# KIYOYOZU/SPH-Poiseuille-Flow

Hardware: AMD Instinct MI355X
Metric: particle-steps/s (higher is better)
Workload: dtype f64; 1 GPU; C2: dp=0.025, DL=3.0, DH=1.0, n_fluid=4800, n_wall=960, n_total=5760, c_f=15.0, transport_coeff=0.3; start=developed (analytic parabola + 0.05dp jitter, seed 12345); lanes_per_particle=16, steps_per_graph=40, rebuild_every=16, forced_rebuilds=0, parallelism=1 GPU, device-resident loop, hipGraph replay

## Files before the change

### sph-poiseuille-flow_amd/csrc/sphx_kernels.hpp

```cpp
#pragma once
#include <type_traits>

#include "sphx_device.hpp"

namespace sphx {

constexpr int kBlock = 256;
constexpr int kScanBlock = 1024;
constexpr int kBigScanCells = 8192;

struct Grid {
    int ncx, ncy, ncells;
    int periodic;
    double DL, half_DL;
    double x0, y0, inv_csx, inv_csy;
    double own_lo, own_hi;
    int own_by_cell, own_c0, own_c1;
};

__device__ __forceinline__ bool owns(const Grid &g, double x, int cell)
{
    if (!g.own_by_cell) return x >= g.own_lo && x < g.own_hi;
    const int cx = cell / g.ncy;
    return cx >= g.own_c0 && cx < g.own_c1;
// ... 38 lines not shown
    double *drhon;
    double4 *a;
    double4 *B;
    double2 *fp, *f;
    double *rho_out, *p_out;
    int *cellid, *count, *perm, *src_of;
    double *vpart;
    double *dpart;
    int *nl_idx;
    int *nl_cnt;
    int *flags;
    int *tile_sum;
    int nl_stride, nl_cap;
    int *sl_idx, *sl_cnt;
    int sl_cap;
    double sl_rcut2;
    int cap;
    int n_vpart;
    double half_skin;
    double *vol;
    int *nl_pk, *sl_pk;
    int has_slack;
    double *seal_out;
    int lazy_out;
    int *tmap;
};

constexpr unsigned long long kVpartEmpty = ~0ull;

struct Walls {
    const double2 *pos;
    const double4 *a;
    const int *id;
    const int *start;
    const int *row_any;
    int n;
};

struct Members {
    Clock *clk;
    const Phys *ph;
    long long part;
    int cells;
    int blocks;
    int lanes;
    long long list, slist;
};

template <typename T>
__device__ __forceinline__ T *member_ptr(T *p, long long stride, int m)
{
    return p ? p + stride * m : p;
}

__device__ __forceinline__ FluidSet member_set(const Members &mb, int m, FluidSet s)
{
    s.pos = member_ptr(s.pos, mb.part, m); s.vel = member_ptr(s.vel, mb.part, m);
    s.drho = member_ptr(s.drho, mb.part, m); s.mass = member_ptr(s.mass, mb.part, m);
    s.id = member_ptr(s.id, mb.part, m); s.cell = member_ptr(s.cell, mb.part, m); s.posb = member_ptr(s.posb, mb.part, m);
    s.start = member_ptr(s.start, mb.cells, m);
    return s;
}

__device__ __forceinline__ FluidTmp member_tmp(const Members &mb, int m, FluidTmp t)
{
    const long long P = mb.part;
    t.posn = member_ptr(t.posn, P, m); t.veln = member_ptr(t.veln, P, m); t.drhon = member_ptr(t.drhon, P, m);
    t.a = member_ptr(t.a, P, m); t.B = member_ptr(t.B, P, m); t.fp = member_ptr(t.fp, P, m); t.f = member_ptr(t.f, P, m);
    t.rho_out = member_ptr(t.rho_out, P, m); t.p_out = member_ptr(t.p_out, P, m); t.vol = member_ptr(t.vol, P, m);
    t.cellid = member_ptr(t.cellid, P, m); t.perm = member_ptr(t.perm, P, m); t.src_of = member_ptr(t.src_of, P, m);
    t.count = member_ptr(t.count, (long long)mb.cells, m);
    t.vpart = member_ptr(t.vpart, (long long)mb.blocks, m); t.dpart = member_ptr(t.dpart, (long long)mb.blocks, m);
    t.nl_idx = member_ptr(t.nl_idx, mb.list, m); t.sl_idx = member_ptr(t.sl_idx, mb.slist, m);
    t.nl_cnt = member_ptr(t.nl_cnt, (long long)mb.lanes, m); t.sl_cnt = member_ptr(t.sl_cnt, (long long)mb.lanes, m);
    t.flags = member_ptr(t.flags, 1ll, m);
    t.tile_sum = nullptr;
    return t;
}

__device__ __forceinline__ void cell_of(const Grid &g, double x, double y, int &cx, int &cy)
{
    cx = (int)floor((x - g.x0) * g.inv_csx);
    cx = min(max(cx, 0), g.ncx - 1);
    cy = (int)floor((y - g.y0) * g.inv_csy);
    cy = min(max(cy, 0), g.ncy - 1);
}

// ... 58 lines not shown
__device__ __forceinline__ double dpp_f64(double v)
{
    const int lo = __builtin_amdgcn_mov_dpp(__double2loint(v), CTRL, 0xF, 0xF, true);
    const int hi = __builtin_amdgcn_mov_dpp(__double2hiint(v), CTRL, 0xF, 0xF, true);
    return __hiloint2double(hi, lo);
}
__device__ __forceinline__ double wave_max(double v)
{
    v = fmax(v, dpp_f64<0xB1>(v));
    v = fmax(v, dpp_f64<0x4E>(v));
    v = fmax(v, dpp_f64<0x141>(v));
    v = fmax(v, dpp_f64<0x140>(v));
    v = fmax(v, __shfl_xor(v, 16));
    return fmax(v, __shfl_xor(v, 32));
}
template <int LPP, bool MAX>
__device__ __forceinline__ int group_extreme(int v)
{
    auto pick = [](int a, int b) { return MAX ? max(a, b) : min(a, b); };
    if (LPP >= 2) v = pick(v, __builtin_amdgcn_mov_dpp(v, 0xB1, 0xF, 0xF, true));
    if (LPP >= 4) v = pick(v, __builtin_amdgcn_mov_dpp(v, 0x4E, 0xF, 0xF, true));
    if (LPP >= 8) v = pick(v, __builtin_amdgcn_mov_dpp(v, 0x141, 0xF, 0xF, true));
    if (LPP >= 16) v = pick(v, __builtin_amdgcn_mov_dpp(v, 0x140, 0xF, 0xF, true));
#pragma unroll
    for (int off = LPP / 2; off >= 16; off >>= 1) v = pick(v, __shfl_xor(v, off));
    return v;
}
template <int LPP>
__device__ __forceinline__ double group_sum(double v)
{
// ... 1 lines not shown
    if (LPP >= 4) v += dpp_f64<0x4E>(v);
    if (LPP >= 8) v += dpp_f64<0x141>(v);
    if (LPP >= 16) v += dpp_f64<0x140>(v);
#pragma unroll
    for (int off = LPP / 2; off >= 16; off >>= 1) v += __shfl_xor(v, off);
    return v;
}

__device__ __forceinline__ double tracked_drift2(const Grid &g, const FluidSet &s, int i, double xo, double yo, const double2 pb)
{
    if (g.own_by_cell && !owns(g, 0.0, s.cell[i])) return 0.0;
    const double ddx = min_image(g, xo - pb.x), ddy = yo - pb.y;
    const double d2 = ddx * ddx + ddy * ddy;
    return d2 != d2 ? INFINITY : d2;
}
__device__ __forceinline__ void store_block_drift(const FluidTmp &t, int blk, double d2)
{
    d2 = wave_max(d2);
    __shared__ double s_d2[kBlock / 64];
    if ((threadIdx.x & 63) == 0) s_d2[threadIdx.x >> 6] = d2;
    __syncthreads();
    if (threadIdx.x == 0) {
        double m = s_d2[0];
        for (int k = 1; k < kBlock / 64; ++k) m = fmax(m, s_d2[k]);
        t.dpart[blk] = m;
    }
}

template <int LPP, typename Body>
__device__ __forceinline__ void sweep(const Grid &g, const int *__restrict__ start, int cx, int cy,
                                      int sub, Body &&body)
{
    const int cylo = max(cy - 1, 0), cyhi = min(cy + 1, g.ncy - 1);
#pragma unroll
    for (int ox = -1; ox <= 1; ++ox) {
        int col;
        if (!neighbour_column(g, cx, ox, col)) continue;
        const int base = col * g.ncy;
        const int lo = start[base + cylo], hi = start[base + cyhi + 1];
        for (int k = lo + sub; k < hi; k += LPP) body(k);
// ... 556 lines not shown
    const double4 ai = in_cap ? t.a[i] : make_double4(1.0, 0.0, 0.0, 0.0);
    const double4 Bi = in_cap ? t.B[i] : make_double4(1.0, 0.0, 0.0, 1.0);
    const double mi = in_cap ? s.mass[i] : 1.0;
    const int nn_all = list_rows(kRowsAhead<LPP> ? head.packed : t.nl_cnt[tid]);
    const FirstRows<LPP> first = kRowsAhead<LPP> ? FirstRows<LPP>(head.e0, head.e1) : FirstRows<LPP>(t.nl_idx, t.nl_stride, tid);
    const bool tracked = s.posb != nullptr;
    const double2 pb = (tracked && in_cap && sub == 0) ? s.posb[i] : make_double2(0.0, 0.0);
    const double2 fp_own = (later && in_cap) ? t.fp[i] : make_double2(0.0, 0.0);
    const double2 p_now = (later && in_cap && sub == 0) ? t.posn[i] : make_double2(0.0, 0.0);
    const double dt = kRowsAhead<LPP> ? head.dt : clk->dt;
    const int run_q = kRowsAhead<LPP> ? head.run : clk->run[q], n_now = kRowsAhead<LPP> ? head.n : clk->n;
    if (kRowsAhead<LPP>) requests_issued();
    if (!run_q) return;
    const bool active = i < n_now;
    const double h = ph.kc.h;
    double ax = 0.0, ay = 0.0, ix = 0.0, iy = 0.0, px = 0.0, py = 0.0, d2 = 0.0;
    const double xi = pi.x, yi = pi.y, vxi = vi.x, vyi = vi.y;
    const double Voli = ai.x, p_i = ai.y, rhoh_i = ai.z;
    const double b11i = Bi.x, b12i = Bi.y, b21i = Bi.z, b22i = Bi.w;
    int first_wall = 1 << 20;
    int h_cell = -1;
    double2 pj0 = make_double2(0.0, 0.0), pj1 = pj0;
    double4 aj0 = make_double4(0.0, 0.0, 0.0, 0.0), aj1 = aj0;
    auto fluid_term = [&](const double2 pj, const double2 vj, const double4 aj, const double4 Bj) {
        const auto [r, ex, ey] = pair_geom(min_image(g, xi - pj.x), yi - pj.y);
        const double dW = spline_dW_in(ph.kc, r);
        const double Volj = aj.x;
        const double tx = (b11i + Bj.x) * ex + (b12i + Bj.y) * ey;
        const double ty = (b21i + Bj.z) * ex + (b22i + Bj.w) * ey;
        const double eBe = ex * tx + ey * ty;
        const double vxj = vj.x, vyj = vj.y;
// ... 92 lines not shown
    }
    px = group_sum<LPP>(px);
    py = group_sum<LPP>(py);
    if (active && sub == 0) {
        const double fx = px * Voli, fy = py * Voli;
        const double vxn = vxi + (fpx + fx) * inv_m * dt;
        const double vyn = vyi + (fpy + fy) * inv_m * dt;
        double sx = 0.0, sy = 0.0;
        if (!later) transport_shift(ix, iy, h, ph.tc, sx, sy);
        double xo = later ? p_now.x : xi + sx, yo = later ? p_now.y : yi + sy;
        xo += 0.5 * dt * vxi;
        yo += 0.5 * dt * vyi;
        xo += 0.5 * dt * vxn;
        yo += 0.5 * dt * vyn;
        if (tracked) d2 = tracked_drift2(g, s, i, xo, yo, pb);
        t.posn[i] = make_double2(g.periodic ? wrap_x(xo, ph.DL) : xo, yo);
        t.veln[i] = make_double2(vxn, vyn);
        if (!later) t.fp[i] = make_double2(fpx, fpy);
        t.f[i] = make_double2(fx, fy);
        if (HIST) {
            int cx, cy;
            cell_of(g, g.periodic ? wrap_x(xo, ph.DL) : xo, yo, cx, cy);
            h_cell = cx * g.ncy + cy;
            t.cellid[i] = h_cell;
            if (!rebin_near(g, c_binned, h_cell)) atomicOr(t.flags, 1);
        }
    }
    __shared__ int s_hc[HIST ? kBlock / LPP : 1];
    if (HIST && sub == 0) s_hc[threadIdx.x / LPP] = h_cell;
    store_block_drift(t, blk, d2);
    if (HIST && threadIdx.x < kBlock / LPP) {
        const int c = s_hc[threadIdx.x];
        int same = 0;
        bool first = true;
#pragma unroll
        for (int k = 0; k < kBlock / LPP; ++k) {
            const bool eq = s_hc[k] == c;
            same += eq ? 1 : 0;
            if (eq && k < (int)threadIdx.x) first = false;
        }
        if (c >= 0 && first) atomicAdd(&t.count[c], same);
    }
}
template <int LPP>
__global__ __launch_bounds__(kBlock) void k_forces(const Clock *clk, int q, int shape, int *nl_cnt, int *nl_idx, int nl_stride, int cap,
// ... 751 lines not shown
        const double sx = ph.tc * h * h * lim * ix, sy = ph.tc * h * h * lim * iy;
        double xo = xi + sx, yo = yi + sy;
        xo += 0.5 * dt * vxi;
        yo += 0.5 * dt * vyi;
        xo += 0.5 * dt * vxn;
        yo += 0.5 * dt * vyn;
        if (tracked) d2 = tracked_drift2(g, s, i, xo, yo, pb);
        if (g.periodic) xo = xo >= ph.DL ? xo - ph.DL : (xo < 0.0 ? xo + ph.DL : xo);
        t.posn[i] = make_double2(xo, yo);
        t.veln[i] = make_double2(vxn, vyn);
        if (want_out) {
            t.fp[i] = make_double2(fpx, fpy);
            t.f[i] = make_double2(fx, fy);
        }
    }
    store_block_drift(t, blk, d2);
}

template <int NT>
__device__ __forceinline__ int block_exclusive_scan_t(int v, int &total, int *s_wave )
{
    const int lane = threadIdx.x & 63, wave = threadIdx.x >> 6;
    int inc = v;
#pragma unroll
    for (int off = 1; off < 64; off <<= 1) {
        const int o = __shfl_up(inc, off);
        if (lane >= off) inc += o;
    }
    if (lane == 63) s_wave[wave] = inc;
    __syncthreads();
    if (wave == 0) {
// ... 38 lines not shown
    c.t += c.n_in > 1 ? c.dt * c.n_in : c.dt;
    c.dt_last = c.dt;
    c.step += 1;
    if (c.steps_left > 0) c.steps_left -= 1;
    if (!(c.vmax == c.vmax) || isinf(c.vmax)) c.status = SPHX_ERR_DIVERGED;
    if (flags) c.status = SPHX_ERR_GRID;
    if (n_new >= 0) c.n = n_new;
    c.dt = next_dt(c, ph);
    const int go = loop_continues(c) ? 1 : 0;
    if (q == 0) c.run[1] = go;
    else c.run[0] = go;
    *clk = c;
    if (!go && c.pub) *c.pub = c;
}

__device__ __forceinline__ void continuity_tail(Clock *clk, int q, const Phys &ph, const FluidTmp &t, int nb, int rebuilt = 0)
{
    if (!clk->run[q]) {
        if (threadIdx.x == 0) clk->run[1 - q] = 0;
        return;
    }
    Clock c0;
    int fl = 0;
    if (threadIdx.x == 0) { c0 = *clk; fl = *t.flags; }
    double m = 0.0, d = 0.0;
    int lost = 0;
    const bool track = t.half_skin >= 0.0;
    for (int k = threadIdx.x; k < nb; k += kBlock) {
        if (track) d = fmax(d, t.dpart[k]);
        unsigned long long *slot = reinterpret_cast<unsigned long long *>(&t.vpart[k]);
// ... 43 lines not shown
    m = wave_max(m);
    d = wave_max(d);
    lost = __any(lost) ? 1 : 0;
    __shared__ double s_m[kBlock / 64], s_d[kBlock / 64];
    __shared__ int s_l[kBlock / 64];
    if ((threadIdx.x & 63) == 0) { s_m[threadIdx.x >> 6] = m; s_d[threadIdx.x >> 6] = d; s_l[threadIdx.x >> 6] = lost; }
    __syncthreads();
    if (threadIdx.x == 0) {
        for (int k = 1; k < kBlock / 64; ++k) { m = fmax(m, s_m[k]); d = fmax(d, s_d[k]); lost |= s_l[k]; }
        t.seal_out[0] = lost ? INFINITY : sqrt(m);
        t.seal_out[1] = sqrt(d);
    }
}

constexpr int kFoldAhead = 8;
struct FoldRebin {
    static constexpr int kPer = kFoldCells / kBlock;
    int cnew = 0, id = 0, cold = 0, lo[3] = {0, 0, 0}, n[3] = {0, 0, 0}, hist[kPer], ccell[kFoldAhead], cid[kFoldAhead];
    double mass = 0.0;
    __device__ __forceinline__ int candidates() const { return n[0] + n[1] + n[2]; }
    __device__ __forceinline__ int slot(int v) const { return ranges_index(lo[0], lo[1], lo[2], n[0], n[1], v); }
};
__device__ __forceinline__ void fold_load(FoldRebin &r, const Grid &g, const FluidSet &s, const FluidTmp &t, int i, bool in_cap, bool lead)
{
    r.cnew = in_cap ? t.cellid[i] : 0;
    r.id = in_cap ? s.id[i] : 0;
    r.cold = lead ? s.cell[i] : 0;
    r.mass = lead ? s.mass[i] : 0.0;
#pragma unroll
    for (int j = 0; j < FoldRebin::kPer; ++j) r.hist[j] = t.count[min((int)threadIdx.x * FoldRebin::kPer + j, g.ncells)];
// ... 92 lines not shown
        atomicAdd(&h_win[dcol * kRows + drow], 1);
        return true;
    }
    __device__ __forceinline__ void flush(const Grid &g, const FluidTmp &t, const int *h_win) const
    {
        if (threadIdx.x >= kCells) return;
        const int v = h_win[threadIdx.x];
        if (v) {
            int col = cx0 + (int)threadIdx.x / kRows;
            if (g.periodic) col = col < 0 ? col + g.ncx : (col >= g.ncx ? col - g.ncx : col);
            const int row = r0 + (int)threadIdx.x % kRows;
            atomicAdd(&t.count[col * g.ncy + row], v);
        }
    }
};
template <int LPP, bool WALK, int TILE, bool CODED = false, bool REBIN = false>
__device__ __forceinline__ void continuity_body(Clock *clk, int q, const Grid &g, const Phys &ph, const FluidSet &s,
                                                const FluidTmp &t, const Walls &w, int do_hist, int tail, int bid, int nb,
                                                double2 *c_pos, double2 *c_vel, double *c_vol, int next_half = 0,
                                                const FluidSet &d = FluidSet{})
{
    static_assert(!CODED || (WALK && TILE == kSlotCodes), "slot-coded lists: this pass stages the whole layout");
    static_assert(!REBIN || (!WALK && TILE == 0 && LPP >= 16), "the folded re-binning belongs to the compact kernels");
    const int blk = xcd_block(bid, nb);
    const int tid = blk * kBlock + threadIdx.x;
    const int i = tid / LPP, sub = tid % LPP;
    const bool in_cap = i < t.cap;
    if (WALK && beyond_population<LPP>(clk, t, blk)) {
        if (threadIdx.x == 0 && clk->run[q] && !next_half) {
            if (tail) __hip_atomic_store(reinterpret_cast<unsigned long long *>(&t.vpart[blk]), 0ull, __ATOMIC_RELAXED, __HIP_MEMORY_SCOPE_AGENT);
            else t.vpart[blk] = 0.0;
// ... 9 lines not shown
    }
    const int run_first = head.run, n_first = head.n;
    const double dt_first = head.dt;
    const double2 pi = in_cap ? s.pos[i] : make_double2(0.0, 0.0);
    const double2 vi = in_cap ? t.veln[i] : make_double2(0.0, 0.0);
    const int packed = kAhead ? head.packed : t.nl_cnt[tid];
    const int nn_all = list_rows(packed);
    const FirstRows<LPP> first = kAhead ? FirstRows<LPP>(head.e0, head.e1) : FirstRows<LPP>(WALK ? t.nl_pk : t.nl_idx, t.nl_stride, tid);
    const bool lead = in_cap && sub == 0;
    const double4 a_own = lead ? t.a[i] : make_double4(0.0, 0.0, 0.0, 0.0);
    const double rhoh_i = a_own.z;
    const double2 pn = (lead && (do_hist || REBIN)) ? t.posn[i] : make_double2(0.0, 0.0);
    FoldRebin fold;
    if (REBIN) fold_load(fold, g, s, t, i, in_cap, lead);
    const TileMap layout = (WALK && TILE > 0) ? tile_map_of(t, blk) : TileMap{0, 0, 0, 0, 0, 0};
    const double dt = kAhead ? dt_first : clk->dt;
    const bool want_out = !WALK || step_outputs_wanted(clk, t);
    const int cell_own = (g.own_by_cell && lead) ? s.cell[i] : 0;
    if (kAhead) requests_issued();
    if (REBIN) fold_runs(fold, g, s);
    if (!(kAhead ? run_first : clk->run[q])) return;
    const int n_now = kAhead ? n_first : clk->n;
    const bool active = i < n_now;
    double rate = 0.0;
    const double xi = pi.x, yi = pi.y, vxi = vi.x, vyi = vi.y;
    const bool hist = do_hist == 1 || (do_hist >= 100 && clk->pos_count >= do_hist - 101);
    constexpr bool kHistWindow = WALK && TILE > 0;
    __shared__ int h_win[kHistWindow ? HistWindow::kCells : 1];
    HistWindow window;
    if (kHistWindow && hist) window.open(g, s.cell[min(blk * (kBlock / LPP), max(n_now - 1, 0))], h_win);
    auto publish_vmax = [&]() {
        double v2 = 0.0;
        if (active && sub == 0 && owns(g, xi, cell_own)) {
            v2 = vxi * vxi + vyi * vyi;
            if (v2 != v2) v2 = INFINITY;
        }
        v2 = wave_max(v2);
        __shared__ double s_max[kBlock / 64];
        if ((threadIdx.x & 63) == 0) s_max[threadIdx.x >> 6] = v2;
        __syncthreads();
        if (threadIdx.x == 0 && !next_half) {
            double m = s_max[0];
            for (int k = 1; k < kBlock / 64; ++k) m = fmax(m, s_max[k]);
            if (tail)
                __hip_atomic_store(reinterpret_cast<unsigned long long *>(&t.vpart[blk]), (unsigned long long)__double_as_longlong(m),
                                   __ATOMIC_RELAXED, __HIP_MEMORY_SCOPE_AGENT);
            else
                t.vpart[blk] = m;
        }
    };
    if (!WALK) publish_vmax();
    __shared__ int r_start[REBIN ? kFoldCells + 1 : 1], r_wave[REBIN ? kBlock / 64 + 1 : 1];
    if (REBIN) fold_scan<LPP>(fold, g, s, t, d, bid, sub, r_start, r_wave);
    if (WALK) {
        const int rows = active ? nn_all : 0, rows_fl = active ? list_fluid_rows(packed) : 0;
        struct Nb {
            double2 p, v;
            double vol;
        };
        TileMap tm{0, 0, 0, 0, 0, 0};
        if (TILE > 0) {
            tm = staged_map<LPP>(layout, blk, n_now, TILE);
            stage_tile<TILE>(tm, [&](int k) { return Nb{s.pos[k], t.veln[k], t.vol[k]}; },
                             [&](int sl, const Nb &n) { c_pos[sl] = n.p; c_vel[sl] = n.v; c_vol[sl] = n.vol; });
        }
        auto fetch_near = [&](int e) { return Nb{lds_double2(c_pos, e), lds_double2(c_vel, e), lds_double(c_vol, e)}; };
// ... 80 lines not shown
        }
        if (next_half) {
            double rhoh2, p2;
            half_state(ph, rho, drho_new, dt, rhoh2, p2);
            t.a[i] = make_double4(a_own.x, p2, rhoh2, rho);
        }
        if (REBIN) fold_store(fold, g, t, d, r_start, r_rank, i, pn, vi, drho_new);
        if (hist) {
            int cx, cy;
            cell_of(g, pn.x, pn.y, cx, cy);
            const int c = cx * g.ncy + cy;
            t.cellid[i] = c;
            if (!(kHistWindow && window.count(g, cx, cy, h_win))) atomicAdd(&t.count[c], 1);
        }
    }
    if (WALK) publish_vmax();
    if (kHistWindow && hist) window.flush(g, t, h_win);
}

template <int LPP, bool WALK, int TILE, bool CODED = false>
__global__ __launch_bounds__(kBlock) __attribute__((amdgpu_waves_per_eu(WALK ? 8 : 1))) void k_continuity(Clock *clk, int q, Grid g, Phys ph,
                                                       FluidSet s, FluidTmp t, Walls w, int do_hist, int tail, int next_half)
{
    constexpr int kSlots = TILE > 0 ? TILE : 1;
    __shared__ double2 c_pos[kSlots], c_vel[kSlots];
    __shared__ double c_vol[kSlots];
    const int nb = (int)gridDim.x - (tail ? 1 : 0);
    if (tail && (int)blockIdx.x == nb) {
        if (tail == 2) slab_seal_tail(clk, q, t, nb);
        else continuity_tail(clk, q, ph, t, nb);
        return;
    }
    continuity_body<LPP, WALK, TILE, CODED>(clk, q, g, ph, s, t, w, do_hist, tail, (int)blockIdx.x, nb, c_pos, c_vel, c_vol, next_half);
}

template <int LPP>
__global__ __launch_bounds__(kBlock) void k_continuity_compact(Clock *clk, int q, int shape, int *nl_cnt, int *nl_idx, int nl_stride,
                                                               int cap, double2 *pos, double2 *veln, Grid g, Phys ph, FluidSet s,
                                                               FluidTmp t, Walls w, int do_hist, int next_half)
{
    t.nl_cnt = nl_cnt; t.nl_idx = nl_idx; t.nl_stride = nl_stride; t.cap = cap; s.pos = pos; t.veln = veln;
    const int nb = shape_blocks(shape), tail = shape_flag(shape);
    if (tail && (int)blockIdx.x == nb) {
        if (tail == 2) slab_seal_tail(clk, q, t, nb);
        else continuity_tail(clk, q, ph, t, nb);
        return;
    }
    continuity_body<LPP, false, 0>(clk, q, g, ph, s, t, w, do_hist, tail, (int)blockIdx.x, nb, nullptr, nullptr, nullptr, next_half);
}

template <int LPP>
__global__ __launch_bounds__(kBlock) void k_continuity_rebin(Clock *clk, int q, int shape, int *nl_cnt, int *nl_idx, int nl_stride,
                                                             int cap, double2 *pos, double2 *veln, Grid g, Phys ph, FluidSet s,
                                                             FluidTmp t, Walls w, FluidSet d)
{
    t.nl_cnt = nl_cnt; t.nl_idx = nl_idx; t.nl_stride = nl_stride; t.cap = cap; s.pos = pos; t.veln = veln;
    const int nb = shape_blocks(shape);
    if ((int)blockIdx.x == nb) {
        continuity_tail(clk, q, ph, t, nb, 1);
        return;
    }
    continuity_body<LPP, false, 0, false, true>(clk, q, g, ph, s, t, w, 0, 1, (int)blockIdx.x, nb, nullptr, nullptr, nullptr, 0, d);
}

template <int LPP>
__global__ __launch_bounds__(kBlock) void k_continuity_density(Clock *clk, int q, int shape, int *e_cnt, int *e_idx, int *a_cnt,
                                                               int *a_idx, int e_stride, int a_stride, Grid g, Phys ph, FluidSet s,
                                                               FluidTmp t, Walls w, FluidSet s_next, FluidTmp t_next)
{
    t.nl_cnt = e_cnt; t.nl_idx = e_idx; t.nl_stride = e_stride;
    t_next.sl_cnt = a_cnt; t_next.sl_idx = a_idx; t_next.nl_stride = a_stride;
    const int nb = shape_blocks(shape), with_tail = shape_flag(shape);
    const int b = (int)blockIdx.x;
    if (with_tail && b == 2 * nb) {
        continuity_tail(clk, q, ph, t, nb);
        return;
    }
    if (b < nb) continuity_body<LPP, false, 0>(clk, q, g, ph, s, t, w, 0, with_tail, b, nb, nullptr, nullptr, nullptr);
    else density_body<LPP, 2>(clk, q, g, ph, s_next, t_next, w, b - nb, nb, false);
}

template <int LPP>
__global__ __launch_bounds__(kBlock) void k_continuity_b(Members mb, int q, Grid g, FluidSet s, FluidTmp t, Walls w,
                                                         int do_hist, int tail)
{
    const int m = (int)blockIdx.y;
    Clock *clk = mb.clk + m;
    const Phys ph = mb.ph[m];
    const FluidTmp tm = member_tmp(mb, m, t);
    const int nb = (int)gridDim.x - (tail ? 1 : 0);
    if (tail && (int)blockIdx.x == nb) {
        continuity_tail(clk, q, ph, tm, nb);
        return;
    }
    continuity_body<LPP, false, 0>(clk, q, g, ph, member_set(mb, m, s), tm, w, do_hist, tail, (int)blockIdx.x, nb, nullptr,
                                   nullptr, nullptr);
}
template <int LPP>
__global__ __launch_bounds__(kBlock) void k_continuity_density_b(Members mb, int q, Grid g, FluidSet s, FluidTmp t, Walls w,
                                                                 FluidSet s_next, FluidTmp t_next, int with_tail)
{
    const int m = (int)blockIdx.y;
    Clock *clk = mb.clk + m;
    const Phys ph = mb.ph[m];
    const int nb = ((int)gridDim.x - with_tail) / 2;
    const int b = (int)blockIdx.x;
    if (with_tail && b == 2 * nb) {
        continuity_tail(clk, q, ph, member_tmp(mb, m, t), nb);
        return;
    }
    if (b < nb) continuity_body<LPP, false, 0>(clk, q, g, ph, member_set(mb, m, s), member_tmp(mb, m, t), w, 0, with_tail, b, nb, nullptr, nullptr, nullptr);
    else density_body<LPP, 2>(clk, q, g, ph, member_set(mb, m, s_next), member_tmp(mb, m, t_next), w, b - nb, nb, false);
}

template <int LPP>
__global__ __launch_bounds__(kBlock) void k_continuity_density_w(Clock *clk, int q, Grid g, Phys ph, FluidSet s, FluidTmp t,
                                                                 Walls w, FluidSet s_next, FluidTmp t_next, int with_tail)
{
    const int nb = ((int)gridDim.x - with_tail) / 2;
    const int b = (int)blockIdx.x;
    if (with_tail && b == 2 * nb) {
        continuity_tail(clk, q, ph, t, nb);
        return;
    }
    if (b < nb) continuity_body<LPP, true, 0>(clk, q, g, ph, s, t, w, 0, with_tail, b, nb, nullptr, nullptr, nullptr);
    else density_walk_body<LPP>(clk, q, g, ph, s_next, t_next, w, b - nb, nb, false);
// ... 147 lines not shown
                                                           const int *flags, const int *count,
                                                           int *start_next, int n_scan, const int *n_new,
                                                           const double *dpart, int rebuilt, double half_skin,
                                                           int *slab_counters, unsigned long long *vpart_reset, int dyn_K)
{
    clock_scan_body(clk, q, ph, n_vpart, vpart, vmax_global, flags, count, start_next, n_scan, n_new, dpart, rebuilt, half_skin,
                    slab_counters, vpart_reset, dyn_K);
}
__global__ __launch_bounds__(kScanBlock) void k_clock_scan_b(Members mb, int q, const double *vpart, const int *flags,
                                                             const int *count, int *start_next, int n_scan,
                                                             const double *dpart, int rebuilt, double half_skin,
                                                             unsigned long long *vpart_reset)
{
    const int m = (int)blockIdx.y;
    const Phys ph = mb.ph[m];
    clock_scan_body(mb.clk + m, q, ph, mb.blocks, member_ptr(vpart, (long long)mb.blocks, m), nullptr, member_ptr(flags, 1ll, m),
                    member_ptr(count, (long long)mb.cells, m), member_ptr(start_next, (long long)mb.cells, m), n_scan, nullptr,
                    member_ptr(dpart, (long long)mb.blocks, m), rebuilt, half_skin, nullptr,
                    member_ptr(vpart_reset, (long long)mb.blocks, m), 0);
}

__global__ __launch_bounds__(kScanBlock) void k_scan_only(const Clock *clk, int q, const int *count, int *start, int n)
{
    if (clk && !slot_active(clk, q)) return;
    scan_counts(count, start, n);
}

__device__ __forceinline__ void scatter_body(const Clock *clk, int q, int n_fixed, const int *cellid, int *count,
                                             const int *start_next, int *perm)
{
    if (clk && !slot_active(clk, q)) return;
    const int n = clk ? clk->n : n_fixed;
    const int lane = threadIdx.x & 63;
    const unsigned long long below = lane ? (~0ull >> (64 - lane)) : 0ull;
// ... 752 lines not shown
```

### sph-poiseuille-flow_amd/csrc/sphx_resident.hip

```cpp
#include <dlfcn.h>
#include <rccl/rccl.h>

#include <algorithm>
#include <array>
#include <cmath>
#include <cstdlib>
#include <limits>
#include <map>

#include "sphx_common.hpp"
#include "sphx_kernels.hpp"
#include "sphx_sampler_state.hpp"

namespace sphx {

struct KernelTimer {
    std::vector<std::string> names;
    std::vector<double> total_ms;
    std::vector<int64_t> launches;
    struct Pending { int idx; hipEvent_t a, b; };
    std::vector<Pending> pending;
    std::vector<Pending> graph_evs;
    bool warned = false, timer_log = false;
    int index_of(const char *name)
// ... 176 lines not shown
    History hist;
    FieldMap fmap;

    sphx::BatchArena *arena = nullptr;
    int member = 0;
    const int *out_ids = nullptr;
    const Members *members = nullptr;
    int n_members = 1;

    FluidSet view(int q, int l)
    {
        return FluidSet{fpos_[q].get(), fvel_[q].get(), fdrho_[q].get(), fmass_[l].get(), fid_[l].get(),
                        fstart_[l].get(), fcell_[l].get(), skin > 0.0 ? fposb_[l].get() : nullptr};
    }
    double half_skin() const { return 0.5 * skin; }
    unsigned long long *vpart_reset() const
    {
        return tail_clock ? reinterpret_cast<unsigned long long *>(vpart.get()) : nullptr;
    }

    ~sphx_ctx()
    {
        if (stream) (void)hipStreamSynchronize(stream);
        sched.drop_graphs();
        if (steps_graph) (void)hipGraphExecDestroy(steps_graph);
        if (ev_fork) (void)hipEventDestroy(ev_fork);
        if (ev_join) (void)hipEventDestroy(ev_join);
        timer.collect();
        timer.drop_graph_events();
        if (ev_computed) (void)hipEventDestroy(ev_computed);
        if (ev_received) (void)hipEventDestroy(ev_received);
        if (stream2) (void)hipStreamSynchronize(stream2);
        if (ev_cd) (void)hipEventDestroy(ev_cd);
// ... 812 lines not shown
{
    const Grid &g = c->grid;
    c->cap = cap;
    c->n_blocks_particles = (int)div_up((size_t)cap * c->lpp, kBlock);
    c->n_blocks_flat = (int)div_up((size_t)cap, kBlock);
    for (int k = 0; k < 2; ++k) {
        dev_alloc(c, c->fpos_[k], cap); dev_alloc(c, c->fvel_[k], cap); dev_alloc(c, c->fdrho_[k], cap); dev_alloc(c, c->fmass_[k], cap);
        dev_alloc(c, c->fid_[k], cap); dev_alloc(c, c->fstart_[k], (size_t)g.ncells + 1); dev_alloc(c, c->fcell_[k], cap);
        if (c->skin > 0.0) dev_alloc(c, c->fposb_[k], cap);
    }
    dev_alloc(c, c->posn, cap); dev_alloc(c, c->veln, cap); dev_alloc(c, c->ffp, cap); dev_alloc(c, c->ff, cap); dev_alloc(c, c->fa, cap); dev_alloc(c, c->fB, cap);
    dev_alloc(c, c->drhon, cap); dev_alloc(c, c->rho_out, cap); dev_alloc(c, c->p_out, cap); dev_alloc(c, c->fvol, cap); c->fvol.zero(c->stream);
    c->posn.zero(c->stream); c->veln.zero(c->stream); c->ffp.zero(c->stream); c->ff.zero(c->stream);
    c->fa.zero(c->stream); c->fB.zero(c->stream); c->drhon.zero(c->stream); c->rho_out.zero(c->stream); c->p_out.zero(c->stream);
    c->n_vpart = c->n_blocks_particles;
    dev_alloc(c, c->vpart, c->n_vpart);
    c->tail_clock = c->skin > 0.0 && !c->is_slab && !c->dyn && c->n_vpart <= tail_clock_limit() && !debug_switches().no_tail_clock;
    const bool vpart_flags = c->tail_clock || (c->is_slab && c->rebuild_every > 1);
    SPHX_HIP(hipMemsetAsync(c->vpart.get(), vpart_flags ? 0xFF : 0, (size_t)c->n_vpart * sizeof(double), c->stream));
    dev_alloc(c, c->dpart, c->n_vpart);
    c->dpart.zero(c->stream);
    c->n_vtiles = (!c->is_slab && c->n_vpart > 4 * kMaxTile) ? (int)div_up((size_t)c->n_vpart, kMaxTile) : 0;
    if (c->n_vtiles) dev_alloc(c, c->vtile, 2 * (size_t)c->n_vtiles);
    dev_alloc(c, c->cellid, cap); dev_alloc(c, c->count, (size_t)g.ncells + 1); dev_alloc(c, c->perm, cap); dev_alloc(c, c->src_of, cap);
    c->count.zero(c->stream);
    const int nl_cap = nl_cap_for(c->lpp);
    const size_t stride = (size_t)c->n_blocks_particles * kBlock;
    dev_alloc(c, c->nl_idx, stride * nl_cap);
    dev_alloc(c, c->nl_cnt, stride);
    c->nl_cnt.zero(c->stream);
    const size_t nl_words = (size_t)(nl_cap + 1) / 2;
    if (c->walk_kernels) { dev_alloc(c, c->nl_pk, stride * std::max<size_t>(nl_words, 2)); c->nl_pk.zero(c->stream); }
    const int sl_cap = c->skin > 0.0 ? (3 * nl_cap + 1) / 2 : 0;
    if (sl_cap) {
        dev_alloc(c, c->sl_idx, stride * sl_cap);
        dev_alloc(c, c->sl_cnt, stride);
        c->sl_cnt.zero(c->stream);
        if (c->walk_kernels) { dev_alloc(c, c->sl_pk, stride * std::max<size_t>((size_t)(sl_cap + 1) / 2, 4)); c->sl_pk.zero(c->stream); }
    }
    const double sl_r = 2.0 * c->prm.h + c->skin;
    dev_alloc(c, c->flags, 1);
    c->flags.zero(c->stream);
    c->big_scan = g.ncells > kBigScanCells;
    c->n_tiles = (int)div_up((size_t)g.ncells, kScanBlock);
    dev_alloc(c, c->tile, 2 * ((size_t)c->n_tiles + 1));
    c->tmp = FluidTmp{c->posn.get(), c->veln.get(), c->drhon.get(), c->fa.get(), c->fB.get(), c->ffp.get(), c->ff.get(),
                      c->rho_out.get(), c->p_out.get(), c->cellid.get(), c->count.get(), c->perm.get(), c->src_of.get(),
                      c->vpart.get(), c->dpart.get(), c->nl_idx.get(), c->nl_cnt.get(), c->flags.get(), c->tile.get(),
                      (int)stride, nl_cap, c->sl_idx.get(), c->sl_cnt.get(), sl_cap, sl_r * sl_r, cap, c->n_vpart,
                      c->skin > 0.0 ? c->half_skin() : -1.0, c->fvol.get(), c->nl_pk.get(), c->sl_pk.get(), c->is_slab ? 1 : 0, nullptr, 0, nullptr};
    c->tmp.lazy_out = (c->walk_kernels && !debug_switches().no_lazy_out) ? (c->is_slab ? 2 : 1) : 0;
    if (c->walk_kernels) {
        dev_alloc(c, c->tmap, 8 * (size_t)c->n_blocks_particles); c->tmap.zero(c->stream);
        c->tmp.tmap = c->tmap.get();
    }
    c->fuse_ea = c->tail_clock && (c->lpp >= 16 || (c->walk_kernels && !c->lds_tiles_be && c->lpp >= 2)) && !debug_switches().no_fuse_ea;
    c->tmp_par[0] = c->tmp;
    c->tmp_par[1] = c->tmp;
    if (c->fuse_ea) {
        dev_alloc(c, c->fa2, cap); dev_alloc(c, c->fvol2, cap); c->fa2.zero(c->stream); c->fvol2.zero(c->stream);
        dev_alloc(c, c->nl_idx2, stride * nl_cap); dev_alloc(c, c->nl_cnt2, stride); c->nl_cnt2.zero(c->stream);
        c->tmp_par[1].a = c->fa2.get(); c->tmp_par[1].vol = c->fvol2.get();
        c->tmp_par[1].nl_idx = c->nl_idx2.get(); c->tmp_par[1].nl_cnt = c->nl_cnt2.get();
        if (c->walk_kernels) {
// ... 1825 lines not shown
            else if (pass == Pass::CD) launch_pass_cd(c, q, fs, tt);
            else if (pass == Pass::E) launch_pass_e(c, q, fs, tt);
            else {
                const FluidSet o = c->view(1 - q, c->sched.lay);
                launch_fused_ea(c, q, fs, writing_into(tt, o), o, c->tmp_par[1 - q], Tail::None);
            }
        }
        SPHX_HIP(hipStreamEndCapture(c->stream, &g));
        SPHX_HIP(hipGraphInstantiate(&e, g, nullptr, nullptr, 0));
        SPHX_HIP(hipGraphLaunch(e, c->stream));
        SPHX_HIP(hipEventCreate(&a));
        SPHX_HIP(hipEventCreate(&b));
        SPHX_HIP(hipEventRecord(a, c->stream));
        SPHX_HIP(hipGraphLaunch(e, c->stream));
        SPHX_HIP(hipEventRecord(b, c->stream));
        if (c->tail_clock)
            SPHX_HIP(hipMemsetAsync(c->vpart.get(), 0xFF, (size_t)c->n_vpart * sizeof(double), c->stream));
        SPHX_HIP(hipStreamSynchronize(c->stream));
        float ms = 0.f;
        SPHX_HIP(hipEventElapsedTime(&ms, a, b));
        *avg_ms = (double)ms / reps;
        c->have_step_outputs = false;
    } catch (...) {
        c->profiling = prof;
        if (a) (void)hipEventDestroy(a);
        if (b) (void)hipEventDestroy(b);
        if (e) (void)hipGraphExecDestroy(e);
        if (g) (void)hipGraphDestroy(g);
        throw;
    }
    c->profiling = prof;
// ... 8 lines not shown
```

Measured before the change: 401.3 million particle-steps/s.

## Compute per-block velocity maxima in the CD pass and simplify the clock tail

```diff
diff --git a/sph-poiseuille-flow_amd/csrc/sphx_kernels.hpp b/sph-poiseuille-flow_amd/csrc/sphx_kernels.hpp
--- a/sph-poiseuille-flow_amd/csrc/sphx_kernels.hpp
+++ b/sph-poiseuille-flow_amd/csrc/sphx_kernels.hpp
@@ -1,4 +1,5 @@
 #pragma once
+#include <cstddef>
 #include <type_traits>
 
 #include "sphx_device.hpp"
@@ -76,6 +77,7 @@
     int nl_stride, nl_cap;
     int *sl_idx, *sl_cnt;
     int sl_cap;
+    int cd_vmax;
     double sl_rcut2;
     int cap;
     int n_vpart;
@@ -88,6 +90,7 @@
     int *tmap;
 };
 
+static_assert(offsetof(FluidTmp, sl_rcut2) == offsetof(FluidTmp, sl_cap) + 8, "cd_vmax sits in the padding behind sl_cap");
 constexpr unsigned long long kVpartEmpty = ~0ull;
 
 struct Walls {
@@ -109,6 +112,7 @@
     long long list, slist;
 };
 
+__device__ __forceinline__ long long maxima_stride(const Members &mb) { return (long long)mb.blocks + 1; }
 template <typename T>
 __device__ __forceinline__ T *member_ptr(T *p, long long stride, int m)
 {
@@ -132,7 +136,7 @@
     t.rho_out = member_ptr(t.rho_out, P, m); t.p_out = member_ptr(t.p_out, P, m); t.vol = member_ptr(t.vol, P, m);
     t.cellid = member_ptr(t.cellid, P, m); t.perm = member_ptr(t.perm, P, m); t.src_of = member_ptr(t.src_of, P, m);
     t.count = member_ptr(t.count, (long long)mb.cells, m);
-    t.vpart = member_ptr(t.vpart, (long long)mb.blocks, m); t.dpart = member_ptr(t.dpart, (long long)mb.blocks, m);
+    t.vpart = member_ptr(t.vpart, maxima_stride(mb), m); t.dpart = member_ptr(t.dpart, maxima_stride(mb), m);
     t.nl_idx = member_ptr(t.nl_idx, mb.list, m); t.sl_idx = member_ptr(t.sl_idx, mb.slist, m);
     t.nl_cnt = member_ptr(t.nl_cnt, (long long)mb.lanes, m); t.sl_cnt = member_ptr(t.sl_cnt, (long long)mb.lanes, m);
     t.flags = member_ptr(t.flags, 1ll, m);
@@ -221,6 +225,17 @@
     v = fmax(v, __shfl_xor(v, 16));
     return fmax(v, __shfl_xor(v, 32));
 }
+__device__ __forceinline__ void wave_max2(double &a, double &b)
+{
+    a = fmax(a, dpp_f64<0xB1>(a));    b = fmax(b, dpp_f64<0xB1>(b));
+    a = fmax(a, dpp_f64<0x4E>(a));    b = fmax(b, dpp_f64<0x4E>(b));
+    a = fmax(a, dpp_f64<0x141>(a));   b = fmax(b, dpp_f64<0x141>(b));
+    a = fmax(a, dpp_f64<0x140>(a));   b = fmax(b, dpp_f64<0x140>(b));
+    const double a16 = __shfl_xor(a, 16), b16 = __shfl_xor(b, 16);
+    a = fmax(a, a16);                 b = fmax(b, b16);
+    const double a32 = __shfl_xor(a, 32), b32 = __shfl_xor(b, 32);
+    a = fmax(a, a32);                 b = fmax(b, b32);
+}
 template <int LPP, bool MAX>
 __device__ __forceinline__ int group_extreme(int v)
 {
@@ -252,16 +267,33 @@
     const double d2 = ddx * ddx + ddy * ddy;
     return d2 != d2 ? INFINITY : d2;
 }
-__device__ __forceinline__ void store_block_drift(const FluidTmp &t, int blk, double d2)
-{
-    d2 = wave_max(d2);
-    __shared__ double s_d2[kBlock / 64];
-    if ((threadIdx.x & 63) == 0) s_d2[threadIdx.x >> 6] = d2;
+__device__ __forceinline__ double speed2(double vx, double vy) { return fma(vx, vx, vy * vy); }
+__device__ __forceinline__ double owned_speed2(const Grid &g, const FluidSet &s, int i, double x, double vx, double vy)
+{
+    if (!owns(g, x, g.own_by_cell ? s.cell[i] : 0)) return 0.0;
+    const double v2 = speed2(vx, vy);
+    return v2 != v2 ? INFINITY : v2;
+}
+template <bool VMAX>
+__device__ __forceinline__ void store_block_maxima(const FluidTmp &t, int blk, double d2, double v2, bool store_v)
+{
+    if (VMAX) wave_max2(d2, v2);
+    else d2 = wave_max(d2);
+    __shared__ double s_mx[VMAX ? 2 : 1][kBlock / 64];
+    if ((threadIdx.x & 63) == 0) {
+        s_mx[0][threadIdx.x >> 6] = d2;
+        if (VMAX) s_mx[VMAX ? 1 : 0][threadIdx.x >> 6] = v2;
+    }
     __syncthreads();
     if (threadIdx.x == 0) {
-        double m = s_d2[0];
-        for (int k = 1; k < kBlock / 64; ++k) m = fmax(m, s_d2[k]);
+        double m = s_mx[0][0];
+        for (int k = 1; k < kBlock / 64; ++k) m = fmax(m, s_mx[0][k]);
         t.dpart[blk] = m;
+        if (VMAX && store_v) {
+            double mv = s_mx[VMAX ? 1 : 0][0];
+            for (int k = 1; k < kBlock / 64; ++k) mv = fmax(mv, s_mx[VMAX ? 1 : 0][k]);
+            t.vpart[blk] = mv;
+        }
     }
 }
 
@@ -848,7 +880,7 @@
     if (!run_q) return;
     const bool active = i < n_now;
     const double h = ph.kc.h;
-    double ax = 0.0, ay = 0.0, ix = 0.0, iy = 0.0, px = 0.0, py = 0.0, d2 = 0.0;
+    double ax = 0.0, ay = 0.0, ix = 0.0, iy = 0.0, px = 0.0, py = 0.0, d2 = 0.0, v2 = 0.0;
     const double xi = pi.x, yi = pi.y, vxi = vi.x, vyi = vi.y;
     const double Voli = ai.x, p_i = ai.y, rhoh_i = ai.z;
     const double b11i = Bi.x, b12i = Bi.y, b21i = Bi.z, b22i = Bi.w;
@@ -971,6 +1003,7 @@
         xo += 0.5 * dt * vxn;
         yo += 0.5 * dt * vyn;
         if (tracked) d2 = tracked_drift2(g, s, i, xo, yo, pb);
+        v2 = owned_speed2(g, s, i, xi, vxn, vyn);
         t.posn[i] = make_double2(g.periodic ? wrap_x(xo, ph.DL) : xo, yo);
         t.veln[i] = make_double2(vxn, vyn);
         if (!later) t.fp[i] = make_double2(fpx, fpy);
@@ -985,7 +1018,8 @@
     }
     __shared__ int s_hc[HIST ? kBlock / LPP : 1];
     if (HIST && sub == 0) s_hc[threadIdx.x / LPP] = h_cell;
-    store_block_drift(t, blk, d2);
+    store_block_maxima<true>(t, blk, d2, v2, t.cd_vmax != 0);
+    if (t.cd_vmax && blk == 0 && threadIdx.x == 0) t.vpart[nblk] = dt;
     if (HIST && threadIdx.x < kBlock / LPP) {
         const int c = s_hc[threadIdx.x];
         int same = 0;
@@ -1767,7 +1801,7 @@
             t.f[i] = make_double2(fx, fy);
         }
     }
-    store_block_drift(t, blk, d2);
+    store_block_maxima<false>(t, blk, d2, 0.0, false);
 }
 
 template <int NT>
@@ -1836,6 +1870,32 @@
     if (!go && c.pub) *c.pub = c;
 }
 
+__device__ __forceinline__ void clock_tail(Clock *clk, int q, const Phys &ph, const FluidTmp &t, int nb, int rebuilt = 0)
+{
+    SPHX_ARGS_BATCH("s"(t.vpart), "s"(t.dpart), "s"(t.flags), "s"(t.half_skin));
+    const int k0 = (int)threadIdx.x;
+    double m = k0 < nb ? t.vpart[k0] : 0.0;
+    double d = k0 < nb ? t.dpart[k0] : 0.0;
+    const int run = clk->run[q];
+    Clock c0;
+    int fl = 0;
+    if (threadIdx.x == 0) { c0 = *clk; fl = *t.flags; }
+    requests_issued();
+    if (!run) {
+        if (threadIdx.x == 0) clk->run[1 - q] = 0;
+        return;
+    }
+    for (int k = k0 + kBlock; k < nb; k += kBlock) { m = fmax(m, t.vpart[k]); d = fmax(d, t.dpart[k]); }
+    wave_max2(m, d);
+    __shared__ double s_m[kBlock / 64], s_d[kBlock / 64];
+    if ((threadIdx.x & 63) == 0) { s_m[threadIdx.x >> 6] = m; s_d[threadIdx.x >> 6] = d; }
+    __syncthreads();
+    if (threadIdx.x == 0) {
+        for (int k = 1; k < kBlock / 64; ++k) { m = fmax(m, s_m[k]); d = fmax(d, s_d[k]); }
+        clock_step(clk, c0, q, ph, sqrt(m), fl, -1, t.half_skin >= 0.0 ? sqrt(d) : -1.0, rebuilt, t.half_skin);
+    }
+}
+
 __device__ __forceinline__ void continuity_tail(Clock *clk, int q, const Phys &ph, const FluidTmp &t, int nb, int rebuilt = 0)
 {
     if (!clk->run[q]) {
@@ -1909,6 +1969,7 @@
 }
 
 constexpr int kFoldAhead = 8;
+constexpr int kPubNever = 0, kPubAlways = 1, kPubUnlessCd = 2;
 struct FoldRebin {
     static constexpr int kPer = kFoldCells / kBlock;
     int cnew = 0, id = 0, cold = 0, lo[3] = {0, 0, 0}, n[3] = {0, 0, 0}, hist[kPer], ccell[kFoldAhead], cid[kFoldAhead];
@@ -2031,7 +2092,7 @@
         }
     }
 };
-template <int LPP, bool WALK, int TILE, bool CODED = false, bool REBIN = false>
+template <int LPP, bool WALK, int TILE, bool CODED = false, bool REBIN = false, int PUB = kPubAlways>
 __device__ __forceinline__ void continuity_body(Clock *clk, int q, const Grid &g, const Phys &ph, const FluidSet &s,
                                                 const FluidTmp &t, const Walls &w, int do_hist, int tail, int bid, int nb,
                                                 double2 *c_pos, double2 *c_vel, double *c_vol, int next_half = 0,
@@ -2071,9 +2132,11 @@
     FoldRebin fold;
     if (REBIN) fold_load(fold, g, s, t, i, in_cap, lead);
     const TileMap layout = (WALK && TILE > 0) ? tile_map_of(t, blk) : TileMap{0, 0, 0, 0, 0, 0};
-    const double dt = kAhead ? dt_first : clk->dt;
+    const bool publishes = PUB == kPubAlways || (PUB == kPubUnlessCd && !t.cd_vmax);
+    const double dt_cd = PUB != kPubAlways ? t.vpart[nb] : 0.0;
+    const double dt = (PUB != kPubAlways && !publishes) ? dt_cd : (kAhead ? dt_first : clk->dt);
     const bool want_out = !WALK || step_outputs_wanted(clk, t);
-    const int cell_own = (g.own_by_cell && lead) ? s.cell[i] : 0;
+    const int cell_own = (PUB != kPubNever && g.own_by_cell && lead) ? s.cell[i] : 0;
     if (kAhead) requests_issued();
     if (REBIN) fold_runs(fold, g, s);
     if (!(kAhead ? run_first : clk->run[q])) return;
@@ -2089,7 +2152,7 @@
     auto publish_vmax = [&]() {
         double v2 = 0.0;
         if (active && sub == 0 && owns(g, xi, cell_own)) {
-            v2 = vxi * vxi + vyi * vyi;
+            v2 = speed2(vxi, vyi);
             if (v2 != v2) v2 = INFINITY;
         }
         v2 = wave_max(v2);
@@ -2106,7 +2169,7 @@
                 t.vpart[blk] = m;
         }
     };
-    if (!WALK) publish_vmax();
+    if (!WALK && publishes) publish_vmax();
     __shared__ int r_start[REBIN ? kFoldCells + 1 : 1], r_wave[REBIN ? kBlock / 64 + 1 : 1];
     if (REBIN) fold_scan<LPP>(fold, g, s, t, d, bid, sub, r_start, r_wave);
     if (WALK) {
@@ -2217,7 +2280,8 @@
             if (!(kHistWindow && window.count(g, cx, cy, h_win))) atomicAdd(&t.count[c], 1);
         }
     }
-    if (WALK) publish_vmax();
+    if (WALK && publishes) publish_vmax();
+    else if (kHistWindow && hist) __syncthreads();
     if (kHistWindow && hist) window.flush(g, t, h_win);
 }
 
@@ -2246,10 +2310,11 @@
     const int nb = shape_blocks(shape), tail = shape_flag(shape);
     if (tail && (int)blockIdx.x == nb) {
         if (tail == 2) slab_seal_tail(clk, q, t, nb);
-        else continuity_tail(clk, q, ph, t, nb);
+        else clock_tail(clk, q, ph, t, nb);
         return;
     }
-    continuity_body<LPP, false, 0>(clk, q, g, ph, s, t, w, do_hist, tail, (int)blockIdx.x, nb, nullptr, nullptr, nullptr, next_half);
+    continuity_body<LPP, false, 0, false, false, kPubUnlessCd>(clk, q, g, ph, s, t, w, do_hist, tail, (int)blockIdx.x, nb, nullptr, nullptr,
+                                                               nullptr, next_half);
 }
 
 template <int LPP>
@@ -2260,10 +2325,10 @@
     t.nl_cnt = nl_cnt; t.nl_idx = nl_idx; t.nl_stride = nl_stride; t.cap = cap; s.pos = pos; t.veln = veln;
     const int nb = shape_blocks(shape);
     if ((int)blockIdx.x == nb) {
-        continuity_tail(clk, q, ph, t, nb, 1);
+        clock_tail(clk, q, ph, t, nb, 1);
         return;
     }
-    continuity_body<LPP, false, 0, false, true>(clk, q, g, ph, s, t, w, 0, 1, (int)blockIdx.x, nb, nullptr, nullptr, nullptr, 0, d);
+    continuity_body<LPP, false, 0, false, true, kPubNever>(clk, q, g, ph, s, t, w, 0, 1, (int)blockIdx.x, nb, nullptr, nullptr, nullptr, 0, d);
 }
 
 template <int LPP>
@@ -2276,10 +2341,10 @@
     const int nb = shape_blocks(shape), with_tail = shape_flag(shape);
     const int b = (int)blockIdx.x;
     if (with_tail && b == 2 * nb) {
-        continuity_tail(clk, q, ph, t, nb);
+        clock_tail(clk, q, ph, t, nb);
         return;
     }
-    if (b < nb) continuity_body<LPP, false, 0>(clk, q, g, ph, s, t, w, 0, with_tail, b, nb, nullptr, nullptr, nullptr);
+    if (b < nb) continuity_body<LPP, false, 0, false, false, kPubNever>(clk, q, g, ph, s, t, w, 0, with_tail, b, nb, nullptr, nullptr, nullptr);
     else density_body<LPP, 2>(clk, q, g, ph, s_next, t_next, w, b - nb, nb, false);
 }
 
@@ -2293,10 +2358,10 @@
     const FluidTmp tm = member_tmp(mb, m, t);
     const int nb = (int)gridDim.x - (tail ? 1 : 0);
     if (tail && (int)blockIdx.x == nb) {
-        continuity_tail(clk, q, ph, tm, nb);
+        clock_tail(clk, q, ph, tm, nb);
         return;
     }
-    continuity_body<LPP, false, 0>(clk, q, g, ph, member_set(mb, m, s), tm, w, do_hist, tail, (int)blockIdx.x, nb, nullptr,
+    continuity_body<LPP, false, 0, false, false, kPubUnlessCd>(clk, q, g, ph, member_set(mb, m, s), tm, w, do_hist, tail, (int)blockIdx.x, nb, nullptr,
                                    nullptr, nullptr);
 }
 template <int LPP>
@@ -2309,10 +2374,10 @@
     const int nb = ((int)gridDim.x - with_tail) / 2;
     const int b = (int)blockIdx.x;
     if (with_tail && b == 2 * nb) {
-        continuity_tail(clk, q, ph, member_tmp(mb, m, t), nb);
+        clock_tail(clk, q, ph, member_tmp(mb, m, t), nb);
         return;
     }
-    if (b < nb) continuity_body<LPP, false, 0>(clk, q, g, ph, member_set(mb, m, s), member_tmp(mb, m, t), w, 0, with_tail, b, nb, nullptr, nullptr, nullptr);
+    if (b < nb) continuity_body<LPP, false, 0, false, false, kPubNever>(clk, q, g, ph, member_set(mb, m, s), member_tmp(mb, m, t), w, 0, with_tail, b, nb, nullptr, nullptr, nullptr);
     else density_body<LPP, 2>(clk, q, g, ph, member_set(mb, m, s_next), member_tmp(mb, m, t_next), w, b - nb, nb, false);
 }
 
@@ -2490,10 +2555,10 @@
 {
     const int m = (int)blockIdx.y;
     const Phys ph = mb.ph[m];
-    clock_scan_body(mb.clk + m, q, ph, mb.blocks, member_ptr(vpart, (long long)mb.blocks, m), nullptr, member_ptr(flags, 1ll, m),
+    clock_scan_body(mb.clk + m, q, ph, mb.blocks, member_ptr(vpart, maxima_stride(mb), m), nullptr, member_ptr(flags, 1ll, m),
                     member_ptr(count, (long long)mb.cells, m), member_ptr(start_next, (long long)mb.cells, m), n_scan, nullptr,
-                    member_ptr(dpart, (long long)mb.blocks, m), rebuilt, half_skin, nullptr,
-                    member_ptr(vpart_reset, (long long)mb.blocks, m), 0);
+                    member_ptr(dpart, maxima_stride(mb), m), rebuilt, half_skin, nullptr,
+                    member_ptr(vpart_reset, maxima_stride(mb), m), 0);
 }
 
 __global__ __launch_bounds__(kScanBlock) void k_scan_only(const Clock *clk, int q, const int *count, int *start, int n)
diff --git a/sph-poiseuille-flow_amd/csrc/sphx_resident.hip b/sph-poiseuille-flow_amd/csrc/sphx_resident.hip
--- a/sph-poiseuille-flow_amd/csrc/sphx_resident.hip
+++ b/sph-poiseuille-flow_amd/csrc/sphx_resident.hip
@@ -214,9 +214,10 @@
                         fstart_[l].get(), fcell_[l].get(), skin > 0.0 ? fposb_[l].get() : nullptr};
     }
     double half_skin() const { return 0.5 * skin; }
+    bool polled_tail() const { return tail_clock && !tmp.cd_vmax; }
     unsigned long long *vpart_reset() const
     {
-        return tail_clock ? reinterpret_cast<unsigned long long *>(vpart.get()) : nullptr;
+        return polled_tail() ? reinterpret_cast<unsigned long long *>(vpart.get()) : nullptr;
     }
 
     ~sphx_ctx()
@@ -1059,11 +1060,13 @@
     c->posn.zero(c->stream); c->veln.zero(c->stream); c->ffp.zero(c->stream); c->ff.zero(c->stream);
     c->fa.zero(c->stream); c->fB.zero(c->stream); c->drhon.zero(c->stream); c->rho_out.zero(c->stream); c->p_out.zero(c->stream);
     c->n_vpart = c->n_blocks_particles;
-    dev_alloc(c, c->vpart, c->n_vpart);
+    const size_t n_maxima = (size_t)c->n_vpart + 1;
+    dev_alloc(c, c->vpart, n_maxima);
     c->tail_clock = c->skin > 0.0 && !c->is_slab && !c->dyn && c->n_vpart <= tail_clock_limit() && !debug_switches().no_tail_clock;
-    const bool vpart_flags = c->tail_clock || (c->is_slab && c->rebuild_every > 1);
-    SPHX_HIP(hipMemsetAsync(c->vpart.get(), vpart_flags ? 0xFF : 0, (size_t)c->n_vpart * sizeof(double), c->stream));
-    dev_alloc(c, c->dpart, c->n_vpart);
+    const bool cd_vmax = !c->is_slab && !c->dyn && c->n_vpart <= tail_clock_limit() && c->lpp >= 16;
+    const bool vpart_flags = (c->tail_clock && !cd_vmax) || (c->is_slab && c->rebuild_every > 1);
+    SPHX_HIP(hipMemsetAsync(c->vpart.get(), vpart_flags ? 0xFF : 0, n_maxima * sizeof(double), c->stream));
+    dev_alloc(c, c->dpart, n_maxima);
     c->dpart.zero(c->stream);
     c->n_vtiles = (!c->is_slab && c->n_vpart > 4 * kMaxTile) ? (int)div_up((size_t)c->n_vpart, kMaxTile) : 0;
     if (c->n_vtiles) dev_alloc(c, c->vtile, 2 * (size_t)c->n_vtiles);
@@ -1092,7 +1095,7 @@
     c->tmp = FluidTmp{c->posn.get(), c->veln.get(), c->drhon.get(), c->fa.get(), c->fB.get(), c->ffp.get(), c->ff.get(),
                       c->rho_out.get(), c->p_out.get(), c->cellid.get(), c->count.get(), c->perm.get(), c->src_of.get(),
                       c->vpart.get(), c->dpart.get(), c->nl_idx.get(), c->nl_cnt.get(), c->flags.get(), c->tile.get(),
-                      (int)stride, nl_cap, c->sl_idx.get(), c->sl_cnt.get(), sl_cap, sl_r * sl_r, cap, c->n_vpart,
+                      (int)stride, nl_cap, c->sl_idx.get(), c->sl_cnt.get(), sl_cap, cd_vmax ? 1 : 0, sl_r * sl_r, cap, c->n_vpart,
                       c->skin > 0.0 ? c->half_skin() : -1.0, c->fvol.get(), c->nl_pk.get(), c->sl_pk.get(), c->is_slab ? 1 : 0, nullptr, 0, nullptr};
     c->tmp.lazy_out = (c->walk_kernels && !debug_switches().no_lazy_out) ? (c->is_slab ? 2 : 1) : 0;
     if (c->walk_kernels) {
@@ -2948,7 +2951,7 @@
         SPHX_HIP(hipEventRecord(a, c->stream));
         SPHX_HIP(hipGraphLaunch(e, c->stream));
         SPHX_HIP(hipEventRecord(b, c->stream));
-        if (c->tail_clock)
+        if (c->polled_tail())
             SPHX_HIP(hipMemsetAsync(c->vpart.get(), 0xFF, (size_t)c->n_vpart * sizeof(double), c->stream));
         SPHX_HIP(hipStreamSynchronize(c->stream));
         float ms = 0.f;
```

Result: no change. 398.8 million particle-steps/s (-0.6%).
